# jibo27/3DGS_Hierarchical_Training

Measured on AMD Instinct MI355X. Metric: train-step images/sec + fwd+bwd ms @1M Gaussians, 980x545; 1/2/4/8 GPU, higher is better.
Workload: dtype f32

## Files before the change

### 3dgs_hierarchical_training_amd/csrc/gsr_kernels.hip

```cpp
#include <hip/hip_runtime.h>
#include <hip/hip_ext.h>
#include <type_traits>
#include <stdint.h>
#include <stdio.h>
#include <string.h>

#include <algorithm>
#include <atomic>
#include <chrono>
#include <cmath>
#include <map>
#include <mutex>
#include <tuple>
#include <vector>

#include "../../include/gsr.h"
#include "gsr_math.h"
#include "adam_math.h"
#include "radix_sort.h"
#include "blend_common.h"

#ifndef GSR_K9_UNROLL
#define GSR_K9_UNROLL 2
#endif
// ... 1073 lines not shown
#pragma unroll
        for (int g = 0; g < kDbMaxGroups; g++) v[g] = g < db.G ? db.GT[(size_t)g * db.Tp + t] : 0u;
#pragma unroll
        for (int g = 0; g < kDbMaxGroups; g++) {
            if (g < db.G) db.GT[(size_t)g * db.Tp + t] = tot;
            tot += v[g];
        }
    }
    if (t >= db.T) tot = 0u;
    const uint32_t inc = wave_inclusive_sum(tot);
    if (lane == 63) s_w[wave] = inc;
    __syncthreads();
    lo = s_lo[0] + s_lo[1] + s_lo[2] + s_lo[3];
    all = s_all[0] + s_all[1] + s_all[2] + s_all[3];
    uint32_t add = 0u;
#pragma unroll
    for (int w = 0; w < 4; w++) add += w < wave ? s_w[w] : 0u;
    const uint32_t base_t = (uint32_t)min(lo + add + inc - tot, 0xffffffffull);
    if (t < db.T) db.tbase[t] = base_t;
    if (cut.key) {
        if (t < db.T) {
            const uint32_t e = cut.cur[0] < (uint32_t)kVcEntries ? cut.cur[0] : 0u;
            const bool use = cut.enable && cut.cur[9] != 0u && cut.owner_n[e] == (uint32_t)db.N;
            uint32_t ck = (uint32_t)(db.NC - 1);
            const uint32_t k = use ? cut.key[(size_t)e * db.T + t] : kCutOpenKey;
            if (k != kCutOpenKey && k != 0u) {
                const float d = __uint_as_float(k);
                const uint32_t kc = __float_as_uint(fmaf(d, cut.margin, d));
                int a = 0, b = db.NC;
                while (a < b) { const int m = (a + b) >> 1; if (s_bkey[m] <= kc) a = m + 1; else b = m; }
                ck = (uint32_t)max(a - 1, 0);
            }
            cut.chunk[t] = (uint16_t)ck;
            cut.flag[t] = 0u;
            if (use) atomicAdd(&cut.hist[ck], 1u);
            if (t == 0) cut.ctl[3] = use ? 1u : 0u;
        }
    }
    if (slab == 0 && tid == 0) {
        db.tbase[db.T] = (uint32_t)min(all, 0xffffffffull);
        *total_out = all;
        if (host_out) {
            __atomic_store_n(host_out + 2, (unsigned long long)g_onesweep_giveups, __ATOMIC_RELAXED);
            __atomic_store_n(host_out + 3, (unsigned long long)(window_overflow ? *window_overflow : 0u), __ATOMIC_RELAXED);
            __atomic_store_n(host_out, all, __ATOMIC_RELAXED);
            __threadfence_system();
            __atomic_store_n(host_out + 1, host_seq, __ATOMIC_RELAXED);
            __threadfence_system();
        }
        if (late_out) scan_report_late(late_out, all, host_seq);
    }
}

constexpr int kDbPairs = 1024;
__device__ __forceinline__ void lds_order() { __builtin_amdgcn_fence(__ATOMIC_ACQ_REL, "wavefront"); __builtin_amdgcn_wave_barrier(); }

__device__ __forceinline__ uint32_t cut_frame(const ListCut& cut, const int NC, uint32_t& deep)
{
    const int lane = threadIdx.x & 63;
    deep = 0u;
    if (cut.ctl[3] == 0u) return (uint32_t)(NC - 1);
    constexpr int kR = 32;
    uint32_t v[kR];
#pragma unroll
    for (int q = 0; q < kR; q++) { const int c = NC - 1 - 64 * q - lane; v[q] = (64 * q < NC && c >= 0) ? cut.hist[c] : 0u; }
    uint32_t acc = 0u;
#pragma unroll
    for (int q = 0; q < kR; q++) {
        if (64 * q >= NC) break;
        const int c = NC - 1 - 64 * q - lane;
        const uint32_t inc = acc + wave_inclusive_sum(v[q]);
        const unsigned long long over = __ballot(c >= 0 && inc > (uint32_t)cut.dmax);
        if (over) {
            const int l = (int)__builtin_ctzll(over);
            deep = (uint32_t)__builtin_amdgcn_readlane((int)(inc - v[q]), l);
            return (uint32_t)(NC - 1 - 64 * q - l);
        }
        acc = (uint32_t)__builtin_amdgcn_readlane((int)inc, 63);
    }
    for (int top = NC - 1 - 64 * kR; top >= 0; top -= 64) {
        const int c = top - lane;
        const uint32_t w = c >= 0 ? cut.hist[c] : 0u;
        const uint32_t inc = acc + wave_inclusive_sum(w);
        const unsigned long long over = __ballot(c >= 0 && inc > (uint32_t)cut.dmax);
        if (over) {
            const int l = (int)__builtin_ctzll(over);
            deep = (uint32_t)__builtin_amdgcn_readlane((int)(inc - w), l);
            return (uint32_t)(top - l);
        }
        acc = (uint32_t)__builtin_amdgcn_readlane((int)inc, 63);
    }
    deep = acc;
    return 0u;
}

template <typename Want>
__device__ __forceinline__ void cut_chunk_tiles(const DirectBin& db, const int c, const int W, const int H, const int tiles_x, const int tiles_y,
                                                const uint32_t* __restrict__ sorted_gid, const TileRec* __restrict__ sorted_rec,
                                                const Splat* __restrict__ splat, uint32_t* __restrict__ list, const uint32_t cap,
                                                uint32_t* s_txy , uint32_t* s_pos , Want&& want)
{
    const int lane = threadIdx.x & 63;
    const unsigned long long lt = lanemask_lt();
    const int j0 = c * db.S, j1 = min(db.N, j0 + db.S);
    const uint32_t* gt = db.GT + (size_t)(c / db.Cg) * db.Tp;
    const uint16_t* mr = db.M + (size_t)c * db.Tp;
    auto load_rec = [&](int j) -> TileRec { TileRec r; r.mask = 0u; r.rect = 1u << 24; if (j < j1) r = sorted_rec[j]; return r; };
// ... 22 lines not shown
        }
        if (nt == 0) break;
        lds_order();
        TileRec rA = load_rec(j0 + lane), rB = load_rec(j0 + 64 + lane);
        uint32_t gA = load_gid(j0 + lane), gB = load_gid(j0 + 64 + lane);
        for (int j = j0; j < j1; j += 64) {
            const TileRec r = rA;
            const uint32_t g = gA;
            rA = rB; gA = gB;
            rB = load_rec(j + 128 + lane);
            gB = load_gid(j + 128 + lane);
            const bool big = (r.rect & kTileRecBig) != 0u && r.mask != 0u;
            const uint32_t ww = (r.rect >> 24) & 63u, rx0 = r.rect & 0xfffu, ry0 = (r.rect >> 12) & 0xfffu;
            TileTest tt = {};
            int bx0 = 0, by0 = 0, bx1 = 0, by1 = 0;
            if (big) {
                const Splat sp = splat[g];
                tile_rect_tight(sp.px, sp.py, sp.radius, sp.ca, sp.cb, sp.cc, sp.op, W, H, tiles_x, tiles_y, bx0, by0, bx1, by1);
                tt = make_tile_test(sp.px, sp.py, sp.ca, sp.cb, sp.cc, sp.op);
            }
            const bool any_big = __ballot(big) != 0ull;
            for (int k = 0; k < nt; k++) {
                const uint32_t txy = s_txy[k], tx = txy & 0xffffu, ty = txy >> 16;
                const uint32_t dx = tx - rx0, dy = ty - ry0, bit = dy * ww + dx;
                bool in = !big && dx < ww && bit < 32u && ((r.mask >> bit) & 1u) != 0u;
                if (any_big && big) in = (int)tx >= bx0 && (int)tx < bx1 && (int)ty >= by0 && (int)ty < by1 && tile_accept(tt, (int)tx, (int)ty, W, H);
                const unsigned long long b = __ballot(in);
                if (b == 0ull) continue;
                const uint32_t p0 = s_pos[k];
                if (in) { const uint32_t pos = p0 + (uint32_t)__popcll(b & lt); if (pos < cap) list[pos] = g; }
                lds_order();
                if (lane == 0) s_pos[k] = p0 + (uint32_t)__popcll(b);
                lds_order();
            }
        }
        lds_order();
    }
}

#ifdef GSR_DB_TIMING
__device__ unsigned long long g_db_dbg[16];
#define DB_T(k) do { const unsigned long long now_ = __builtin_readcyclecounter(); if (lane == 0) dbt[k] += now_ - dbt_last; dbt_last = now_; } while (0)
#else
#define DB_T(k) do { } while (0)
#endif
template <bool SLAB, bool PAIRS = false, int CUT = 0>
__global__ __launch_bounds__(64) void k_chunk_scatter(DirectBin db, int W, int H, int tiles_x, int tiles_y,
                                                      const uint32_t* __restrict__ sorted_gid, const TileRec* __restrict__ sorted_rec,
                                                      const Splat* __restrict__ splat, uint32_t* __restrict__ list, uint2* __restrict__ ranges,
                                                      uint32_t cap, const uint32_t* __restrict__ dkey = nullptr, uint2* __restrict__ pairs = nullptr,
                                                      ListCut cut = ListCut{})
{
    static_assert(!CUT || (!SLAB && !PAIRS), "the list cut serves the plain direct binning");
    extern __shared__ unsigned long long s_dyn[];
    const int LT = SLAB ? db.Tsp : db.Tp;
    unsigned long long* const s_mask = s_dyn;
    uint32_t* const s_cnt = reinterpret_cast<uint32_t*>(s_dyn + LT);
    uint32_t* const s_pair = s_cnt + LT;
    const int lane = threadIdx.x, b = (int)blockIdx.x;
    if (CUT == 2 && cut.ctl[2] == 0u) return;
    uint32_t cstar = 0u, ndeep = 0u;
    if (CUT == 1) cstar = cut_frame(cut, db.NC, ndeep);
    if (CUT == 2) cstar = cut.ctl[0];
    {
        const int t = b * 64 + lane;
        if (t < db.T) {
            uint32_t tend = db.tbase[t + 1];
            if (CUT == 1) {
                const uint32_t c1 = max((uint32_t)cut.chunk[t], cstar) + 1u;
                if (c1 < (uint32_t)db.NC) tend = db.tbase[t] + db.GT[(size_t)(c1 / (uint32_t)db.Cg) * db.Tp + t] + (uint32_t)db.M[(size_t)c1 * db.Tp + t];
                cut.tend[t] = tend;
            }
            const uint32_t lo = min(db.tbase[t], cap), hi = min(tend, cap);
            if (CUT != 2 || cut.flag[t]) ranges[t] = hi > lo ? make_uint2(lo, hi) : make_uint2(0u, 0u);
            if (CUT == 1) {
                const uint32_t e = cut.cur[0] < (uint32_t)kVcEntries ? cut.cur[0] : 0u;
                cut.key[(size_t)e * db.T + t] = 0u;
            }
        }
        if (CUT && b == 0 && lane == 0) {
            if (CUT == 1) {
                const uint32_t e = cut.cur[0] < (uint32_t)kVcEntries ? cut.cur[0] : 0u;
                cut.owner_n[e] = (uint32_t)db.N;
                cut.ctl[0] = cstar; cut.ctl[1] = ndeep;
                cut.stats[0] += 1u;
                cut.stats[3] += (uint32_t)(db.NC - 1) - min(cstar, (uint32_t)(db.NC - 1));
                cut.stats[4] += ndeep;
            } else { cut.stats[1] += 1u; cut.stats[2] += cut.ctl[2]; }
        }
    }
    const int per = (db.NC + 7) >> 3, kk = b >> 3, c = (b & 7) * per + (SLAB ? kk / db.NS : kk), slab = SLAB ? kk % db.NS : 0;
    if ((SLAB ? kk / db.NS : kk) >= per || c >= db.NC) return;
    if (CUT && (uint32_t)c > cstar) {
        if (CUT == 1 && ndeep == 0u) return;
        uint32_t* const s_tile = s_pair;
        uint32_t* const s_pos = s_pair + 64;
        if (CUT == 1) cut_chunk_tiles(db, c, W, H, tiles_x, tiles_y, sorted_gid, sorted_rec, splat, list, cap, s_tile, s_pos,
                                      [&](uint32_t t) { return (uint32_t)cut.chunk[t] >= (uint32_t)c; });
        else cut_chunk_tiles(db, c, W, H, tiles_x, tiles_y, sorted_gid, sorted_rec, splat, list, cap, s_tile, s_pos,
                             [&](uint32_t t) { return cut.flag[t] != 0u && (uint32_t)cut.chunk[t] < (uint32_t)c; });
        return;
    }
    if (CUT == 2) return;
    const uint32_t t0 = SLAB ? (uint32_t)(slab * db.Ts) : 0u;
    const uint32_t tn = SLAB ? (uint32_t)min(db.Ts, db.T - slab * db.Ts) : (uint32_t)db.T;
    const int srow0 = slab * db.slab_rows, srow1 = srow0 + db.slab_rows;
#ifdef GSR_DB_TIMING
    unsigned long long dbt[8] = {0, 0, 0, 0, 0, 0, 0, 0}, dbt_last = __builtin_readcyclecounter();
#endif
    {
        const uint32_t* gt = db.GT + (size_t)(c / db.Cg) * db.Tp;
        const uint16_t* mr = db.M + (size_t)c * db.Tp;
        constexpr int kRows = 36;
        for (int i0 = 0; i0 < LT; i0 += 64 * kRows) {
            uint32_t tb[kRows], gb[kRows], mc[kRows];
#pragma unroll
            for (int q = 0; q < kRows; q++) {
                const int i = i0 + 64 * q + lane;
                const bool v = i < LT && (uint32_t)i < tn + (SLAB ? 0u : (uint32_t)(db.Tp - db.T));
                const int g = (int)t0 + i;
                tb[q] = v && g < db.T ? db.tbase[g] : 0u;
                gb[q] = v ? gt[g] : 0u;
                mc[q] = v ? (uint32_t)mr[g] : 0u;
            }
#pragma unroll
            for (int q = 0; q < kRows; q++) {
                const int i = i0 + 64 * q + lane;
                if (i < LT) { s_cnt[i] = tb[q] + gb[q] + mc[q]; s_mask[i] = 0ull; }
            }
        }
    }
    lds_order();
    DB_T(0);
    const unsigned long long me = 1ull << lane, lt = lanemask_lt();
    const int j0 = c * db.S, j1 = min(db.N, j0 + db.S);
    auto load_gid = [&](int j) -> uint32_t { return j < j1 ? (PAIRS ? (uint32_t)j : sorted_gid[j]) : 0u; };
    auto load_rec = [&](int j) -> TileRec { TileRec r; r.mask = 0u; r.rect = 1u << 24; if (j < j1) r = sorted_rec[j]; return r; };
    auto load_key = [&](int j) -> uint32_t { return (PAIRS && j < j1) ? dkey[j] : 0u; };
    uint32_t gA = load_gid(j0 + lane), gB = load_gid(j0 + 64 + lane);
    TileRec rA = load_rec(j0 + lane), rB = load_rec(j0 + 64 + lane);
    uint32_t kA = load_key(j0 + lane), kB = load_key(j0 + 64 + lane);
    for (int j = j0 + lane; j - lane < j1; j += 64) {
        const uint32_t g = gA;
        TileRec r = rA;
        const uint32_t kd = kA;
        gA = gB; rA = rB; kA = kB;
        gB = load_gid(j + 128);
        rB = load_rec(j + 128);
        kB = load_key(j + 128);
        if (SLAB && !(r.rect & kTileRecBig)) {
            const int ww = (int)((r.rect >> 24) & 63u), ry0 = (int)((r.rect >> 12) & 0xfffu);
            const int lo = min(32, max(0, (srow0 - ry0) * ww)), hi = min(32, max(0, (srow1 - ry0) * ww));
            const uint32_t below_hi = hi >= 32 ? 0xffffffffu : ((1u << hi) - 1u), below_lo = lo >= 32 ? 0xffffffffu : ((1u << lo) - 1u);
            r.mask &= below_hi & ~below_lo;
        }
        const bool big = (r.rect & kTileRecBig) != 0u && r.mask != 0u, huge = big && (SLAB || r.mask > (uint32_t)kDbPairs);
        const unsigned long long bigs = __ballot(big && !huge), huges = __ballot(huge);
        const uint32_t cnt = huge ? 0u : tilerec_count(r);
        const uint32_t incl = wave_inclusive_sum(cnt);
        auto run_end = [&](int lo, uint32_t before) -> int {
            const unsigned long long over = __ballot(incl - before > (uint32_t)kDbPairs) & ~((1ull << lo) - 1ull);
            return over ? (int)__builtin_ctzll(over) : 64;
        };
        auto owners = [&](int lo, int hi, uint32_t before, bool with_or) {
            const bool mine = lane >= lo && lane < hi;
            if (!big && (with_or || mine)) {
                uint32_t* o = s_pair + (incl - cnt - before);
                small_rect_tiles(r, tiles_x, [&](uint32_t tg) {
                    const uint32_t t = tg - t0;
                    if (with_or) atomicOr(&s_mask[t], me);
                    if (mine) *o++ = (t << 6) | (uint32_t)lane;
                });
            }
            for (unsigned long long bm = bigs; bm != 0ull; bm &= bm - 1ull) {
                const int bl = (int)__builtin_ctzll(bm);
                const bool in_run = bl >= lo && bl < hi;
                if (!with_or && !in_run) continue;
                const uint32_t gg = (uint32_t)__builtin_amdgcn_readlane((int)g, bl), rect = (uint32_t)__builtin_amdgcn_readlane((int)r.rect, bl);
                uint32_t o = (uint32_t)__builtin_amdgcn_readlane((int)(incl - cnt), bl) - before;
                const Splat s = splat[gg];
                big_rect_tiles(s, rect, W, H, tiles_x, tiles_y, lane, [&](bool ok, uint32_t tg) {
                    const uint32_t t = tg - t0;
                    const unsigned long long acc = __ballot(ok);
                    if (ok) {
                        if (with_or) atomicOr(&s_mask[t], 1ull << bl);
                        if (in_run) s_pair[(o + (uint32_t)__popcll(acc & lt)) & (uint32_t)(kDbPairs - 1)] = (t << 6) | (uint32_t)bl;
                    }
                    o += (uint32_t)__popcll(acc);
                });
            }
        };
        int lo = 0, hi = run_end(0, 0u);
        uint32_t before = 0u;
        const bool one_run = hi == 64;
        DB_T(1);
        owners(0, hi, 0u, true);
        DB_T(2);
        for (unsigned long long bm = huges; bm != 0ull; bm &= bm - 1ull) {
            const int bl = (int)__builtin_ctzll(bm);
            const uint32_t gg = (uint32_t)__builtin_amdgcn_readlane((int)g, bl), rect = (uint32_t)__builtin_amdgcn_readlane((int)r.rect, bl);
            const Splat s = splat[gg];
            big_rect_tiles(s, rect, W, H, tiles_x, tiles_y, lane, [&](bool ok, uint32_t tg) { const uint32_t t = tg - t0; if (ok && t < tn) atomicOr(&s_mask[t], 1ull << bl); });
        }
        asm volatile("" : "+v"(gA), "+v"(rA.mask), "+v"(rA.rect));
        if (PAIRS) asm volatile("" : "+v"(kA));
        lds_order();
        DB_T(3);
        for (;;) {
            const uint32_t P = (uint32_t)__builtin_amdgcn_readlane((int)incl, hi - 1) - before;
            for (uint32_t p0 = 0u; p0 < P; p0 += 512u) {
                const uint32_t left = P - p0;
                auto batch = [&](auto rounds_tag) {
                    constexpr int RN = decltype(rounds_tag)::value;
                    uint32_t e[RN], go[RN], base[RN], ko[PAIRS ? RN : 1];
                    unsigned long long mk[RN];
#pragma unroll
                    for (int q = 0; q < RN; q++) e[q] = s_pair[(p0 + 64u * q + (uint32_t)lane) & (uint32_t)(kDbPairs - 1)];
#pragma unroll
                    for (int q = 0; q < RN; q++) {
                        const bool v = 64u * q + (uint32_t)lane < left;
                        e[q] = v ? e[q] : 0xffffffffu;
                        const uint32_t t = v ? e[q] >> 6 : 0u;
                        go[q] = (uint32_t)__builtin_amdgcn_ds_bpermute((int)((e[q] & 63u) << 2), (int)g);
                        if (PAIRS) ko[q] = (uint32_t)__builtin_amdgcn_ds_bpermute((int)((e[q] & 63u) << 2), (int)kd);
                        mk[q] = s_mask[t];
                        base[q] = s_cnt[t];
                    }
#pragma unroll
                    for (int q = 0; q < RN; q++)
                        if (e[q] != 0xffffffffu) {
                            const uint32_t pos = base[q] + (uint32_t)__popcll(mk[q] & ((1ull << (e[q] & 63u)) - 1ull));
                            if (pos < cap) {
                                if (PAIRS) pairs[pos] = make_uint2(ko[q], go[q]);
                                else list[pos] = go[q];
                            }
                        }
                };
                if (left <= 128u) batch(std::integral_constant<int, 2>{});
                else if (left <= 256u) batch(std::integral_constant<int, 4>{});
                else if (left <= 384u) batch(std::integral_constant<int, 6>{});
                else batch(std::integral_constant<int, 8>{});
            }
            if (hi == 64) break;
            lds_order();
            before += P;
            lo = hi;
            hi = run_end(lo, before);
            owners(lo, hi, before, false);
            lds_order();
        }
        for (unsigned long long bm = huges; bm != 0ull; bm &= bm - 1ull) {
            const int bl = (int)__builtin_ctzll(bm);
            const uint32_t gg = (uint32_t)__builtin_amdgcn_readlane((int)g, bl), rect = (uint32_t)__builtin_amdgcn_readlane((int)r.rect, bl);
            const Splat s = splat[gg];
            big_rect_tiles(s, rect, W, H, tiles_x, tiles_y, lane, [&](bool ok, uint32_t tg) {
                const uint32_t t = tg - t0;
                if (ok && t < tn) {
                    const uint32_t pos = s_cnt[t] + (uint32_t)__popcll(s_mask[t] & ((1ull << bl) - 1ull));
                    if (pos < cap) {
                        if (PAIRS) pairs[pos] = make_uint2((uint32_t)__builtin_amdgcn_readlane((int)kd, bl), gg);
                        else list[pos] = gg;
                    }
                }
            });
        }
        lds_order();
        DB_T(4);
        if (one_run) {
            const uint32_t P = (uint32_t)__builtin_amdgcn_readlane((int)incl, 63);
            for (uint32_t p0 = 0u; p0 < P; p0 += 512u) {
                const uint32_t left = P - p0;
                auto batch = [&](auto rounds_tag) {
                    constexpr int RN = decltype(rounds_tag)::value;
                    uint32_t e[RN];
#pragma unroll
                    for (int q = 0; q < RN; q++) e[q] = s_pair[(p0 + 64u * q + (uint32_t)lane) & (uint32_t)(kDbPairs - 1)];
#pragma unroll
                    for (int q = 0; q < RN; q++)
                        if (64u * q + (uint32_t)lane < left) { atomicAdd(&s_cnt[e[q] >> 6], 1u); s_mask[e[q] >> 6] = 0ull; }
                };
                if (left <= 128u) batch(std::integral_constant<int, 2>{});
                else if (left <= 256u) batch(std::integral_constant<int, 4>{});
                else if (left <= 384u) batch(std::integral_constant<int, 6>{});
                else batch(std::integral_constant<int, 8>{});
            }
        } else {
            if (!big) small_rect_tiles(r, tiles_x, [&](uint32_t tg) { const uint32_t t = tg - t0; atomicAdd(&s_cnt[t], 1u); s_mask[t] = 0ull; });
            for (unsigned long long bm = bigs; bm != 0ull; bm &= bm - 1ull) {
                const int bl = (int)__builtin_ctzll(bm);
                const uint32_t gg = (uint32_t)__builtin_amdgcn_readlane((int)g, bl), rect = (uint32_t)__builtin_amdgcn_readlane((int)r.rect, bl);
                const Splat s = splat[gg];
                big_rect_tiles(s, rect, W, H, tiles_x, tiles_y, lane, [&](bool ok, uint32_t tg) { const uint32_t t = tg - t0; if (ok && t < tn) { atomicAdd(&s_cnt[t], 1u); s_mask[t] = 0ull; } });
            }
        }
        for (unsigned long long bm = huges; bm != 0ull; bm &= bm - 1ull) {
            const int bl = (int)__builtin_ctzll(bm);
            const uint32_t gg = (uint32_t)__builtin_amdgcn_readlane((int)g, bl), rect = (uint32_t)__builtin_amdgcn_readlane((int)r.rect, bl);
            const Splat s = splat[gg];
            big_rect_tiles(s, rect, W, H, tiles_x, tiles_y, lane, [&](bool ok, uint32_t tg) { const uint32_t t = tg - t0; if (ok && t < tn) { atomicAdd(&s_cnt[t], 1u); s_mask[t] = 0ull; } });
        }
        lds_order();
        DB_T(5);
    }
#ifdef GSR_DB_TIMING
    if (lane == 0) {
        for (int k = 0; k < 6; k++) atomicAdd(&g_db_dbg[k], dbt[k]);
        atomicAdd(&g_db_dbg[6], 1ull);
        atomicAdd(&g_db_dbg[7], (unsigned long long)((j1 - j0 + 63) / 64));
    }
#endif
}

constexpr int kTsCap = 4096, kTsSmallMax = 1024;

template <int THREADS, int IPT, bool GATHER = false>
__device__ __forceinline__ void tile_sort_regs(const uint2* __restrict__ src, uint32_t* dst, uint32_t n, const uint32_t* __restrict__ dkey,
                                               unsigned long long (*s_mask)[256], uint32_t (*s_cnt)[256], uint32_t* s_keys, uint32_t* s_vals,
                                               uint32_t* s_start, uint32_t* s_wsum, uint32_t* s_bits)
{
    constexpr int WAVES = THREADS / 64;
    const int tid = threadIdx.x, wave = tid >> 6, lane = tid & 63;
    uint32_t key[IPT], val[IPT], dig[IPT], rnk[IPT];
    uint32_t k_or = 0u, k_and = 0xffffffffu;
#pragma unroll
    for (int r = 0; r < IPT; r++) {
        const uint32_t p = (uint32_t)(wave * (IPT * 64) + r * 64 + lane);
        if (GATHER) val[r] = p < n ? dst[p] : 0u;
        else if (p < n) { const uint2 e = src[p]; key[r] = e.x; val[r] = e.y; }
        if (!GATHER && p >= n) { key[r] = 0xffffffffu; val[r] = 0u; }
    }
    if (GATHER) {
#pragma unroll
        for (int r = 0; r < IPT; r++) {
            const uint32_t p = (uint32_t)(wave * (IPT * 64) + r * 64 + lane);
            key[r] = p < n ? dkey[val[r]] : 0xffffffffu;
        }
    }
#pragma unroll
    for (int r = 0; r < IPT; r++) {
        const uint32_t p = (uint32_t)(wave * (IPT * 64) + r * 64 + lane);
        if (p < n) { k_or |= key[r]; k_and &= key[r]; }
    }
#pragma unroll
    for (int off = 32; off > 0; off >>= 1) { k_or |= (uint32_t)__shfl_xor((int)k_or, off, 64); k_and &= (uint32_t)__shfl_xor((int)k_and, off, 64); }
    if (lane == 0) { s_bits[wave] = k_or; s_bits[WAVES + wave] = k_and; }
    __syncthreads();
    uint32_t differ = 0u;
    {
        uint32_t o = 0u, a = 0xffffffffu;
#pragma unroll
        for (int w = 0; w < WAVES; w++) { o |= s_bits[w]; a &= s_bits[WAVES + w]; }
        differ = o & ~a;
    }
#pragma unroll 1
// ... 2135 lines not shown
    if (!strcmp(name, "tile_sort")) { if (value < 0 || value > 2) return GSR_ERR_ARG; g_tile_sort = value; return GSR_OK; }
    if (!strcmp(name, "tile_sort_max_avg")) { if (value < 0) return GSR_ERR_ARG; g_tile_sort_max_avg = value; return GSR_OK; }
    if (!strcmp(name, "direct_slab_tiles")) { if (value < 0) return GSR_ERR_ARG; g_db_slab_tiles = value; return GSR_OK; }
    if (!strcmp(name, "view_pose_tol_e6")) { if (value < 0) return GSR_ERR_ARG; g_view_pose_tol_e6 = value; return GSR_OK; }
    if (!strcmp(name, "depth_sort9")) { g_depth_sort9 = value ? 1 : 0; return GSR_OK; }
    if (!strcmp(name, "direct_binning")) { g_direct_bin = value ? 1 : 0; return GSR_OK; }
    if (!strcmp(name, "speculative_binning")) { g_speculate = value ? 1 : 0; return GSR_OK; }
    if (!strcmp(name, "deterministic_backward")) { g_deterministic = value ? 1 : 0; return GSR_OK; }
    if (!strcmp(name, "binning_capacity_hint")) {
        std::lock_guard<std::mutex> lk(g_state_mutex);
        g_hint_override = value > 0 ? value : -1;
        return GSR_OK;
    }
    if (!strcmp(name, "reset_speculation")) {
        std::lock_guard<std::mutex> lk(g_state_mutex);
        g_hints.clear(); g_hint_override = -1;
        g_spec_overflows = 0; g_spec_forwards = 0; g_exact_forwards = 0; g_depth_window_resorts = 0;
        g_full_depth_sort.clear();
        return GSR_OK;
    }
    if (!strcmp(name, "profile")) { g_profile = (value == 2 || value == 3) ? value : (value ? 1 : 0); g_profile_tick = 0; return GSR_OK; }
    if (!strcmp(name, "prep_hist_max_n")) { g_prep_hist_max_n = value; return GSR_OK; }
    if (!strcmp(name, "small_sort9")) { if (value < 0) return GSR_ERR_ARG; g_small_sort9 = value; return GSR_OK; }
    if (!strcmp(name, "poll_iters")) { g_poll_iters = value < 0 ? 0 : value; return GSR_OK; }
    if (!strcmp(name, "emit_hist")) { g_emit_hist = value ? 1 : 0; return GSR_OK; }
    if (!strcmp(name, "sort_algo")) { if (value < 0 || value > 2) return GSR_ERR_ARG; g_sort_algo = value; return GSR_OK; }
    if (!strcmp(name, "blend_bwd_ppt")) {
        if (value < 0 || value > 2) return GSR_ERR_ARG;
        g_bwd_ppt = value; return GSR_OK;
    }
    return GSR_ERR_ARG;
}

struct DirectBinScratch { size_t M, GT, tbase, bsum, cut_chunk, cut_tend, cut_flag, cut_ctl, cut_bkey, cut_hist, bytes; };
static bool direct_bin_geometry(int N, int T, DirectBin& db, DirectBinScratch& ds, int tiles_x = 0, int tile_rows = 0)
{
    if (N < 1 || T < 1) return false;
    db.NS = 1; db.Ts = 0; db.Tsp = 0; db.slab_rows = 0;
    static const bool force_slabs = getenv("GSR_DB_FORCE_SLABS") != nullptr;
    if (T > kDbMaxTiles || (force_slabs && g_db_slab_tiles > 0 && tiles_x > 0 && tile_rows > 0 && tiles_x * tile_rows == T)) {
        if (g_db_slab_tiles <= 0 || tiles_x <= 0 || tile_rows <= 0 || tiles_x * tile_rows != T || tiles_x > kDbMaxTiles || T > 32768) return false;
        const int rows = std::max(1, std::min(g_db_slab_tiles, kDbMaxTiles) / tiles_x);
        db.slab_rows = rows; db.Ts = rows * tiles_x; db.Tsp = (db.Ts + 63) & ~63; db.NS = (tile_rows + rows - 1) / rows;
        if (db.NS > 16) return false;
    }
    static std::atomic<int> cus_cached{0};
    int cus = cus_cached.load(std::memory_order_relaxed);
    if (!cus) {
        int dev = 0, n = 0;
        cus = (hipGetDevice(&dev) == hipSuccess && hipDeviceGetAttribute(&n, hipDeviceAttributeMultiprocessorCount, dev) == hipSuccess && n > 0) ? n : 256;
        cus_cached.store(cus, std::memory_order_relaxed);
    }
    db.N = N; db.T = T; db.Tp = (T + 63) & ~63;
    const int lds = 12 * (db.NS > 1 ? db.Tsp : db.Tp) + 4 * kDbPairs;
    const char* env = getenv("GSR_DB_WAVES_PER_CU");
    int per_cu = std::min(16, (160 * 1024) / lds);
    if (env && atoi(env) > 0) per_cu = atoi(env);
    const long long resident = std::max<long long>(1, (long long)cus * per_cu / db.NS);
    const char* env_s = getenv("GSR_DB_MIN_CHUNK");
    const int min_s = env_s && atoi(env_s) > 0 ? atoi(env_s) : 128;
    long long S = ((long long)N + resident - 1) / resident;
    S = std::max<long long>(min_s, (S + 63) & ~63ll);
    if (S > 65472) return false;
    db.S = (int)S;
    db.NC = (int)(((long long)N + S - 1) / S);
    int G = 1;
    while (G * G < db.NC) G++;
    db.Cg = std::max(1, std::min((db.NC + G - 1) / G, 65535 / db.S));
    db.G = (db.NC + db.Cg - 1) / db.Cg;
    if (db.G > kDbMaxGroups) return false;
    size_t o = 0;
    ds.M = o; o += align256((size_t)db.NC * db.Tp * sizeof(uint16_t));
    ds.GT = o; o += align256((size_t)db.G * db.Tp * sizeof(uint32_t));
    ds.tbase = o; o += align256((size_t)(db.Tp + 1) * sizeof(uint32_t));
    ds.bsum = o; o += align256((size_t)db.G * ((db.Tp + 255) / 256) * sizeof(uint32_t));
    ds.cut_chunk = o; o += align256((size_t)db.Tp * sizeof(uint16_t));
    ds.cut_tend = o; o += align256((size_t)db.Tp * sizeof(uint32_t));
    ds.cut_flag = o; o += align256((size_t)db.Tp * sizeof(uint32_t));
    ds.cut_ctl = o; o += 256;
    ds.cut_bkey = o; o += align256((size_t)db.NC * sizeof(uint32_t));
    ds.cut_hist = o; o += align256((size_t)db.NC * sizeof(uint32_t));
    ds.bytes = o;
    return true;
}

int gsr_forward(const GsrForwardArgs* a, GsrForwardOut* out, void* stream_)
{
    CallTimer call_timer(g_fwd_calls, g_fwd_ns);
    hipStream_t st = (hipStream_t)stream_;
    if (!a || !out) return fail(GSR_ERR_ARG, "null args%s");
    int rc = check_common(a->N, a->M, a->D, a->W, a->H);
    if (rc) return rc;
    if (!a->out_color || !a->out_depth || !a->out_alpha || !a->image || !a->bg || !a->alloc)
        return fail(GSR_ERR_ARG, "missing output / workspace pointer%s");
    const int N = a->N, W = a->W, H = a->H;
    BatchDev bt;
    rc = batch_dev(a->batch, N, H, bt);
    if (rc) return rc;
    const int NB = bt.B;
    const int opt_ppt = g_blend_ppt ? g_blend_ppt : 7, opt_map = g_tile_map, opt_ckpt = g_ckpt_first;
    const int tiles_x = (W + kTile - 1) / kTile, tiles_y = (H + kTile - 1) / kTile, T = tiles_x * tiles_y * NB;
    if (NB > 1 && opt_ppt < 6) return fail(GSR_ERR_ARG, "batch: served by the default forward blend kernel only%s");
    if (a->out_color_clamped && opt_ppt < 6) return fail(GSR_ERR_ARG, "out_color_clamped: served by the default forward blend kernel only%s");
    out->num_rendered = 0; out->binning = nullptr; out->binning_bytes = 0; out->binning_capacity = 0;
    out->forward_flags = pack_fwd_flags(opt_ppt, opt_map, opt_ckpt);
    uint64_t R = 0;
    BlendBalance bb = {};
// ... 46 lines not shown
    auto launch_binning_t = [&](auto key_tag, uint64_t capacity, const unsigned long long* n_dev, bool prezeroed) -> int {
        using KeyT = decltype(key_tag);
        if (!prezeroed) GSR_HIP(hipMemsetAsync(ranges, 0, (size_t)T * sizeof(uint2), st));
        if (capacity == 0) return GSR_OK;
        KeyT* tkey = reinterpret_cast<KeyT*>(bs + S.tile);
        KeyT* tkey_alt = reinterpret_cast<KeyT*>(bs + S.tile_alt);
        uint32_t* gid_alt2 = reinterpret_cast<uint32_t*>(bs + S.gid_alt);
        uint32_t* block_sums = reinterpret_cast<uint32_t*>(fs + L.block_sums);
        uint32_t* v0 = (tile_passes & 1) ? gid_alt2 : list;
        uint32_t* v1 = (tile_passes & 1) ? list : gid_alt2;
        const bool emit_hist = g_sort_algo == 2 && prezeroed && g_emit_hist;
        EmitHist eh = {};
        if (emit_hist) {
            eh.ghist = reinterpret_cast<uint32_t*>(bs + S.sort);
            eh.status = onesweep_status(bs + S.sort);
            eh.status_words = onesweep_status_words<KeyT>((uint32_t)capacity, bits);
            eh.bits = bits;
            eh.n_dev = n_dev;
        }
        {
            ProfScope ps(P_EMIT, st);
            hipLaunchKernelGGL(k_emit<KeyT>, dim3(nb), dim3(kEmitThreads), 0, st, N, W, H, tiles_x, tiles_y, sorted_gid, splat,
                               tsort ? ts_rec : reinterpret_cast<const TileRec*>(fs + L.srec), block_sums, tkey, v0,
                               (uint32_t)capacity, eh);
        }
        int in_alt = 0;
        {
            ProfScope ps(P_SORT_TILE, st);
            GSR_HIP(g_sort_algo == 2 ? onesweep_sort_pairs<KeyT>(tkey, v0, tkey_alt, v1, (uint32_t)capacity, 0, bits, bs + S.sort,
                                                                 &in_alt, st, n_dev, prezeroed, emit_hist)
                                     : radix_sort_pairs<KeyT>(tkey, v0, tkey_alt, v1, (uint32_t)capacity, 0, tile_passes * 8, bs + S.sort,
                                                              &in_alt, st));
        }
        const KeyT* skey = in_alt ? tkey_alt : tkey;
        {
            ProfScope ps(P_RANGES, st);
            constexpr uint32_t kpb = 256u * (16u / (uint32_t)sizeof(KeyT));
            hipLaunchKernelGGL(k_tile_ranges<KeyT>, dim3(((uint32_t)capacity + kpb - 1) / kpb), dim3(256), 0, st, (uint32_t)capacity, skey, ranges, n_dev);
        }
        if (tsort) {
            ProfScope ps(P_SORT_DEPTH, st);
            hipLaunchKernelGGL(k_tile_sort_wave<true>, dim3(T), dim3(64), 0, st, ranges, pairs, list, T, ts_dkey);
            hipLaunchKernelGGL((k_tile_sort<1024, true>), dim3(std::min(T, 512)), dim3(1024), 0, st, ranges, pairs, pairs_alt, list, T, ts_dkey);
        }
        return GSR_OK;
    };
    auto launch_binning = [&](uint64_t capacity, const unsigned long long* n_dev, bool prezeroed) -> int {
        if (direct) {
            if (capacity == 0) { GSR_HIP(hipMemsetAsync(ranges, 0, (size_t)T * sizeof(uint2), st)); return GSR_OK; }
            const int per = (db.NC + 7) / 8, grid = std::max(8 * per * db.NS, (T + 63) / 64);
            if (tsort) {
                {
                    ProfScope ps(P_EMIT, st);
                    hipLaunchKernelGGL((k_chunk_scatter<false, true>), dim3(grid), dim3(64), (size_t)12 * db.Tp + 4 * kDbPairs, st, db, W, H, tiles_x, tiles_y,
                                       (const uint32_t*)nullptr, ts_rec, splat, list, ranges, (uint32_t)std::min<uint64_t>(capacity, 0xffffffffull), ts_dkey, pairs);
                }
                ProfScope ps2(P_SORT_TILE, st);
                hipLaunchKernelGGL(k_tile_sort_wave<false>, dim3(T), dim3(64), 0, st, ranges, pairs, list, T, (const uint32_t*)nullptr);
                hipLaunchKernelGGL(k_tile_sort<1024>, dim3(std::min(T, 512)), dim3(1024), 0, st, ranges, pairs, pairs_alt, list, T);
                return GSR_OK;
            }
            ProfScope ps(P_EMIT, st);
            if (db.NS > 1)
                hipLaunchKernelGGL(k_chunk_scatter<true>, dim3(grid), dim3(64), (size_t)12 * db.Tsp + 4 * kDbPairs, st, db, W, H, tiles_x, tiles_y, sorted_gid,
                                   reinterpret_cast<const TileRec*>(fs + L.srec), splat, list, ranges, (uint32_t)std::min<uint64_t>(capacity, 0xffffffffull));
            else if (lc.key) {
                lc_capacity = capacity;
                hipLaunchKernelGGL((k_chunk_scatter<false, false, 1>), dim3(grid), dim3(64), (size_t)12 * db.Tp + 4 * kDbPairs, st, db, W, H,
                                   tiles_x, tiles_y, sorted_gid, reinterpret_cast<const TileRec*>(fs + L.srec), splat, list, ranges,
                                   (uint32_t)std::min<uint64_t>(capacity, 0xffffffffull), (const uint32_t*)nullptr, (uint2*)nullptr, lc);
            } else
                hipLaunchKernelGGL(k_chunk_scatter<false>, dim3(grid), dim3(64), (size_t)12 * db.Tp + 4 * kDbPairs, st, db, W, H, tiles_x, tiles_y, sorted_gid,
                                   reinterpret_cast<const TileRec*>(fs + L.srec), splat, list, ranges, (uint32_t)std::min<uint64_t>(capacity, 0xffffffffull));
            return GSR_OK;
        }
        return wide_keys ? launch_binning_t(uint32_t{}, capacity, n_dev, prezeroed) : launch_binning_t(uint16_t{}, capacity, n_dev, prezeroed);
    };
    auto launch_blend = [&](bool prezeroed) -> int {
        const int ppt = opt_ppt;
        if (!prezeroed) GSR_HIP(hipMemsetAsync(staged, 0, (size_t)T * 16, st));
        float* ckpt = reinterpret_cast<float*>(bin + B.ckpt);
        if (ppt == 7 && g_profile && (g_profile != 3 || g_profile_tick.fetch_add(1u) % 3u == 0u)) {
            hipEvent_t ea = nullptr, eb = nullptr;
            if (hipEventCreate(&ea) != hipSuccess || hipEventCreate(&eb) != hipSuccess) return fail(GSR_ERR_HIP, "hipEventCreate failed%s");
            hipExtLaunchKernelGGL(k_blend_fwd_w6<true>, dim3(8 * 4 * slots_per_xcd(opt_map, T, tiles_x)), dim3(64), 0, st, ea, eb, 0, W, H, tiles_x, T, ranges, list,
                                  splat, a->bg, a->out_color, a->out_depth, a->out_alpha, img, staged, opt_map, ckpt, opt_ckpt, tiles_y, bb, a->out_color_clamped,
                                  lc, lc.key ? 1 : 0);
            std::lock_guard<std::mutex> lk(g_prof_mutex);
            g_prof_events[P_BLEND_FWD].push_back({ea, eb});
        } else {
            ProfScope ps(ppt == 7 && g_profile == 3 ? P_COUNT : P_BLEND_FWD, st);
            if (ppt == 7)
                hipLaunchKernelGGL(k_blend_fwd_w6<true>, dim3(8 * 4 * slots_per_xcd(opt_map, T, tiles_x)), dim3(64), 0, st, W, H, tiles_x, T, ranges, list, splat, a->bg,
                                   a->out_color, a->out_depth, a->out_alpha, img, staged, opt_map, ckpt, opt_ckpt, tiles_y, bb, a->out_color_clamped,
                                   lc, lc.key ? 1 : 0);
            else if (ppt == 6)
                hipLaunchKernelGGL(k_blend_fwd_w6<false>, dim3(8 * 4 * slots_per_xcd(opt_map, T, tiles_x)), dim3(64), 0, st, W, H, tiles_x, T, ranges, list, splat, a->bg,
                                   a->out_color, a->out_depth, a->out_alpha, img, staged, opt_map, ckpt, opt_ckpt, tiles_y, BlendBalance{}, a->out_color_clamped);
            else return fail(GSR_ERR_ARG, "unknown forward blend variant%s");
        }
        if (ppt == 7 && lc.key && lc_capacity > 0) {
            ProfScope ps(P_CUT_REPAIR, st);
            const int per = (db.NC + 7) / 8, grid = std::max(8 * per * db.NS, (T + 63) / 64);
            hipLaunchKernelGGL((k_chunk_scatter<false, false, 2>), dim3(grid), dim3(64), (size_t)12 * db.Tp + 4 * kDbPairs, st, db, W, H,
                               tiles_x, tiles_y, sorted_gid, reinterpret_cast<const TileRec*>(fs + L.srec), splat, list, ranges,
                               (uint32_t)std::min<uint64_t>(lc_capacity, 0xffffffffull), (const uint32_t*)nullptr, (uint2*)nullptr, lc);
            hipLaunchKernelGGL(k_blend_fwd_w6<true>, dim3(8 * 4 * slots_per_xcd(opt_map, T, tiles_x)), dim3(64), 0, st, W, H, tiles_x, T, ranges, list, splat, a->bg,
                               a->out_color, a->out_depth, a->out_alpha, img, staged, opt_map, ckpt, opt_ckpt, tiles_y, bb, a->out_color_clamped, lc, 2);
        }
        GSR_HIP(hipGetLastError());
        return GSR_OK;
    };

    if (N == 0) {
        rc = alloc_binning(0);
        if (rc) return rc;
        rc = launch_binning(0, nullptr, false);
        if (rc) return rc;
        rc = launch_blend(false);
        if (rc) return rc;
        out->binning = bin;
        out->binning_bytes = B.bytes;
        return GSR_OK;
    }

    if (!a->means3D || !a->opacities || !a->geom || !a->radii || !a->viewmatrix || !a->projmatrix)
        return fail(GSR_ERR_ARG, "missing input pointer%s");
    if ((a->shs == nullptr) == (a->colors_precomp == nullptr)) return fail(GSR_ERR_ARG, "provide exactly one of shs / colors_precomp%s");
    if ((a->cov3D_precomp == nullptr) == (a->scales == nullptr || a->rotations == nullptr))
        return fail(GSR_ERR_ARG, "provide exactly one of (scales, rotations) / cov3D_precomp%s");
    if (a->shs && (!a->campos || a->M < (a->D + 1) * (a->D + 1))) return fail(GSR_ERR_ARG, "shs needs campos and M >= (D+1)^2%s");

    int dev_id = 0;
    GSR_HIP(hipGetDevice(&dev_id));
    const auto hint_key = std::make_tuple(dev_id, W, H * NB, n_bucket(N));
    uint64_t hint = 0;
    {
        std::lock_guard<std::mutex> lk(g_state_mutex);
        if (g_hint_override > 0) { hint = (uint64_t)g_hint_override; g_hint_override = -1; }
        else { auto it = g_hints.find(hint_key); if (it != g_hints.end()) hint = it->second; }
    }
    const bool speculative = g_speculate && g_sort_algo == 2 && hint > 0;
    const uint64_t cap = speculative ? hint : 0;
    {
        const int ts_mode = g_tile_sort;
        const uint64_t avg = (hint > 0 ? hint : (uint64_t)N * 4u) / (uint64_t)T;
        const bool auto_ok = ts_mode == 1 && avg <= (uint64_t)g_tile_sort_max_avg && (direct || N / std::max(1, NB) <= g_tile_sort_emit_max_n);
        tsort = (ts_mode == 2 || auto_ok) && g_sort_algo == 2 && (direct ? (NB == 1 && db.NS == 1) : true);
    }

    fs = static_cast<uint8_t*>(a->alloc(align256(L.bytes) + (direct ? dbs.bytes : 0), GSR_ALLOC_SCRATCH, a->alloc_user));
    if (!fs) return fail(GSR_ERR_ALLOC, "scratch allocation failed%s");
    if (speculative) {
        rc = alloc_binning(cap);
        if (rc) return rc;
    }
    uint32_t* dkey = reinterpret_cast<uint32_t*>(fs + L.dkey);
// ... 644 lines not shown
```

Before: 1206.

## Use 32-bit per-tile lane masks and per-run half-wave placement in chunk scatter

The direct-binning scatter kernel replaces its 64-bit per-tile lane mask with a 32-bit mask and processes each run of pairs in two half-wave passes. The OR-mask is now built inside each run rather than once for the whole wave. The pair buffer shrinks from 1024 to 512 entries, and the per-workgroup LDS footprint drops from 12*LT+4K to 8*LT+2K bytes. The intent is higher occupancy (more waves per CU) and cheaper 32-bit LDS atomics, at the cost of extra barriers and a repeated huge-splat tile walk per half.

```diff
diff --git a/3dgs_hierarchical_training_amd/csrc/gsr_kernels.hip b/3dgs_hierarchical_training_amd/csrc/gsr_kernels.hip
--- a/3dgs_hierarchical_training_amd/csrc/gsr_kernels.hip
+++ b/3dgs_hierarchical_training_amd/csrc/gsr_kernels.hip
@@ -1149,7 +1149,8 @@
     }
 }
 
-constexpr int kDbPairs = 1024;
+constexpr int kDbPairs = 512;
+__host__ __device__ constexpr size_t db_scatter_lds(int LT) { return (size_t)8 * LT + 4 * kDbPairs; }
 __device__ __forceinline__ void lds_order() { __builtin_amdgcn_fence(__ATOMIC_ACQ_REL, "wavefront"); __builtin_amdgcn_wave_barrier(); }
 
 __device__ __forceinline__ uint32_t cut_frame(const ListCut& cut, const int NC, uint32_t& deep)
@@ -1278,10 +1279,10 @@
                                                       ListCut cut = ListCut{})
 {
     static_assert(!CUT || (!SLAB && !PAIRS), "the list cut serves the plain direct binning");
-    extern __shared__ unsigned long long s_dyn[];
+    extern __shared__ uint32_t s_dyn[];
     const int LT = SLAB ? db.Tsp : db.Tp;
-    unsigned long long* const s_mask = s_dyn;
-    uint32_t* const s_cnt = reinterpret_cast<uint32_t*>(s_dyn + LT);
+    uint32_t* const s_mask = s_dyn;
+    uint32_t* const s_cnt = s_dyn + LT;
     uint32_t* const s_pair = s_cnt + LT;
     const int lane = threadIdx.x, b = (int)blockIdx.x;
     if (CUT == 2 && cut.ctl[2] == 0u) return;
@@ -1352,13 +1353,13 @@
 #pragma unroll
             for (int q = 0; q < kRows; q++) {
                 const int i = i0 + 64 * q + lane;
-                if (i < LT) { s_cnt[i] = tb[q] + gb[q] + mc[q]; s_mask[i] = 0ull; }
+                if (i < LT) { s_cnt[i] = tb[q] + gb[q] + mc[q]; s_mask[i] = 0u; }
             }
         }
     }
     lds_order();
     DB_T(0);
-    const unsigned long long me = 1ull << lane, lt = lanemask_lt();
+    const unsigned long long lt = lanemask_lt();
     const int j0 = c * db.S, j1 = min(db.N, j0 + db.S);
     auto load_gid = [&](int j) -> uint32_t { return j < j1 ? (PAIRS ? (uint32_t)j : sorted_gid[j]) : 0u; };
     auto load_rec = [&](int j) -> TileRec { TileRec r; r.mask = 0u; r.rect = 1u << 24; if (j < j1) r = sorted_rec[j]; return r; };
@@ -1384,148 +1385,123 @@
         const unsigned long long bigs = __ballot(big && !huge), huges = __ballot(huge);
         const uint32_t cnt = huge ? 0u : tilerec_count(r);
         const uint32_t incl = wave_inclusive_sum(cnt);
+        auto lanes = [](int lo, int hi) -> unsigned long long { return (hi >= 64 ? ~0ull : ((1ull << hi) - 1ull)) & ~((1ull << lo) - 1ull); };
         auto run_end = [&](int lo, uint32_t before) -> int {
             const unsigned long long over = __ballot(incl - before > (uint32_t)kDbPairs) & ~((1ull << lo) - 1ull);
             return over ? (int)__builtin_ctzll(over) : 64;
         };
-        auto owners = [&](int lo, int hi, uint32_t before, bool with_or) {
-            const bool mine = lane >= lo && lane < hi;
-            if (!big && (with_or || mine)) {
+        auto owners = [&](int lo, int hi, uint32_t before) {
+            if (!big && lane >= lo && lane < hi) {
                 uint32_t* o = s_pair + (incl - cnt - before);
-                small_rect_tiles(r, tiles_x, [&](uint32_t tg) {
-                    const uint32_t t = tg - t0;
-                    if (with_or) atomicOr(&s_mask[t], me);
-                    if (mine) *o++ = (t << 6) | (uint32_t)lane;
-                });
-            }
-            for (unsigned long long bm = bigs; bm != 0ull; bm &= bm - 1ull) {
+                small_rect_tiles(r, tiles_x, [&](uint32_t tg) { *o++ = ((tg - t0) << 6) | (uint32_t)lane; });
+            }
+            for (unsigned long long bm = bigs & lanes(lo, hi); bm != 0ull; bm &= bm - 1ull) {
                 const int bl = (int)__builtin_ctzll(bm);
-                const bool in_run = bl >= lo && bl < hi;
-                if (!with_or && !in_run) continue;
                 const uint32_t gg = (uint32_t)__builtin_amdgcn_readlane((int)g, bl), rect = (uint32_t)__builtin_amdgcn_readlane((int)r.rect, bl);
                 uint32_t o = (uint32_t)__builtin_amdgcn_readlane((int)(incl - cnt), bl) - before;
                 const Splat s = splat[gg];
                 big_rect_tiles(s, rect, W, H, tiles_x, tiles_y, lane, [&](bool ok, uint32_t tg) {
                     const uint32_t t = tg - t0;
                     const unsigned long long acc = __ballot(ok);
-                    if (ok) {
-                        if (with_or) atomicOr(&s_mask[t], 1ull << bl);
-                        if (in_run) s_pair[(o + (uint32_t)__popcll(acc & lt)) & (uint32_t)(kDbPairs - 1)] = (t << 6) | (uint32_t)bl;
-                    }
+                    if (ok) s_pair[(o + (uint32_t)__popcll(acc & lt)) & (uint32_t)(kDbPairs - 1)] = (t << 6) | (uint32_t)bl;
                     o += (uint32_t)__popcll(acc);
                 });
             }
         };
-        int lo = 0, hi = run_end(0, 0u);
-        uint32_t before = 0u;
-        const bool one_run = hi == 64;
-        DB_T(1);
-        owners(0, hi, 0u, true);
-        DB_T(2);
-        for (unsigned long long bm = huges; bm != 0ull; bm &= bm - 1ull) {
-            const int bl = (int)__builtin_ctzll(bm);
-            const uint32_t gg = (uint32_t)__builtin_amdgcn_readlane((int)g, bl), rect = (uint32_t)__builtin_amdgcn_readlane((int)r.rect, bl);
-            const Splat s = splat[gg];
-            big_rect_tiles(s, rect, W, H, tiles_x, tiles_y, lane, [&](bool ok, uint32_t tg) { const uint32_t t = tg - t0; if (ok && t < tn) atomicOr(&s_mask[t], 1ull << bl); });
-        }
-        asm volatile("" : "+v"(gA), "+v"(rA.mask), "+v"(rA.rect));
-        if (PAIRS) asm volatile("" : "+v"(kA));
-        lds_order();
-        DB_T(3);
-        for (;;) {
+        auto huge_walk = [&](unsigned long long hm, auto&& f) {
+            for (; hm != 0ull; hm &= hm - 1ull) {
+                const int bl = (int)__builtin_ctzll(hm);
+                const uint32_t gg = (uint32_t)__builtin_amdgcn_readlane((int)g, bl), rect = (uint32_t)__builtin_amdgcn_readlane((int)r.rect, bl);
+                const Splat s = splat[gg];
+                big_rect_tiles(s, rect, W, H, tiles_x, tiles_y, lane, [&](bool ok, uint32_t tg) { const uint32_t t = tg - t0; if (ok && t < tn) f(t, bl, gg); });
+            }
+        };
+        auto place_run = [&](int lo, int hi, uint32_t before) {
             const uint32_t P = (uint32_t)__builtin_amdgcn_readlane((int)incl, hi - 1) - before;
-            for (uint32_t p0 = 0u; p0 < P; p0 += 512u) {
-                const uint32_t left = P - p0;
-                auto batch = [&](auto rounds_tag) {
-                    constexpr int RN = decltype(rounds_tag)::value;
-                    uint32_t e[RN], go[RN], base[RN], ko[PAIRS ? RN : 1];
-                    unsigned long long mk[RN];
-#pragma unroll
-                    for (int q = 0; q < RN; q++) e[q] = s_pair[(p0 + 64u * q + (uint32_t)lane) & (uint32_t)(kDbPairs - 1)];
+            const unsigned long long run = lanes(lo, hi);
+            auto batch = [&](auto rounds_tag) {
+                constexpr int RN = decltype(rounds_tag)::value;
+                uint32_t e[RN], go[RN], ko[PAIRS ? RN : 1];
+#pragma unroll
+                for (int q = 0; q < RN; q++) e[q] = s_pair[(64u * q + (uint32_t)lane) & (uint32_t)(kDbPairs - 1)];
+#pragma unroll
+                for (int q = 0; q < RN; q++) {
+                    e[q] = 64u * q + (uint32_t)lane < P ? e[q] : 0xffffffffu;
+                    go[q] = (uint32_t)__builtin_amdgcn_ds_bpermute((int)((e[q] & 63u) << 2), (int)g);
+                    if (PAIRS) ko[q] = (uint32_t)__builtin_amdgcn_ds_bpermute((int)((e[q] & 63u) << 2), (int)kd);
+                }
+#pragma unroll
+                for (int h = 0; h < 2; h++) {
+                    const unsigned long long half = h ? 0xffffffff00000000ull : 0x00000000ffffffffull;
+                    if ((run & half) == 0ull) continue;
+                    const unsigned long long hm = huges & run & half;
+                    bool act[RN];
+                    uint32_t t[RN], mk[RN], base[RN];
 #pragma unroll
                     for (int q = 0; q < RN; q++) {
-                        const bool v = 64u * q + (uint32_t)lane < left;
-                        e[q] = v ? e[q] : 0xffffffffu;
-                        const uint32_t t = v ? e[q] >> 6 : 0u;
-                        go[q] = (uint32_t)__builtin_amdgcn_ds_bpermute((int)((e[q] & 63u) << 2), (int)g);
-                        if (PAIRS) ko[q] = (uint32_t)__builtin_amdgcn_ds_bpermute((int)((e[q] & 63u) << 2), (int)kd);
-                        mk[q] = s_mask[t];
-                        base[q] = s_cnt[t];
+                        act[q] = e[q] != 0xffffffffu && ((e[q] >> 5) & 1u) == (uint32_t)h;
+                        t[q] = act[q] ? e[q] >> 6 : 0u;
+                        if (act[q]) atomicOr(&s_mask[t[q]], 1u << (e[q] & 31u));
                     }
+                    if (hm) huge_walk(hm, [&](uint32_t tt, int bl, uint32_t) { atomicOr(&s_mask[tt], 1u << (bl & 31)); });
+                    lds_order();
+#pragma unroll
+                    for (int q = 0; q < RN; q++) { mk[q] = s_mask[t[q]]; base[q] = s_cnt[t[q]]; }
 #pragma unroll
                     for (int q = 0; q < RN; q++)
-                        if (e[q] != 0xffffffffu) {
-                            const uint32_t pos = base[q] + (uint32_t)__popcll(mk[q] & ((1ull << (e[q] & 63u)) - 1ull));
+                        if (act[q]) {
+                            const uint32_t pos = base[q] + (uint32_t)__popc(mk[q] & ((1u << (e[q] & 31u)) - 1u));
                             if (pos < cap) {
                                 if (PAIRS) pairs[pos] = make_uint2(ko[q], go[q]);
                                 else list[pos] = go[q];
                             }
                         }
-                };
-                if (left <= 128u) batch(std::integral_constant<int, 2>{});
-                else if (left <= 256u) batch(std::integral_constant<int, 4>{});
-                else if (left <= 384u) batch(std::integral_constant<int, 6>{});
-                else batch(std::integral_constant<int, 8>{});
-            }
-            if (hi == 64) break;
+                    if (hm) {
+                        huge_walk(hm, [&](uint32_t tt, int bl, uint32_t gg) {
+                            const uint32_t pos = s_cnt[tt] + (uint32_t)__popc(s_mask[tt] & ((1u << (bl & 31)) - 1u));
+                            if (pos < cap) {
+                                if (PAIRS) pairs[pos] = make_uint2((uint32_t)__builtin_amdgcn_readlane((int)kd, bl), gg);
+                                else list[pos] = gg;
+                            }
+                        });
+                        lds_order();
+#pragma unroll
+                        for (int q = 0; q < RN; q++)
+                            if (act[q]) { atomicAdd(&s_cnt[t[q]], 1u); s_mask[t[q]] = 0u; }
+                        huge_walk(hm, [&](uint32_t tt, int, uint32_t) { atomicAdd(&s_cnt[tt], 1u); s_mask[tt] = 0u; });
+                    } else {
+                        lds_order();
+#pragma unroll
+                        for (int q = 0; q < RN; q++)
+                            if (act[q] && (mk[q] >> (e[q] & 31u)) == 1u) { s_cnt[t[q]] = base[q] + (uint32_t)__popc(mk[q]); s_mask[t[q]] = 0u; }
+                    }
+                    lds_order();
+                }
+            };
+            static_assert(kDbPairs == 512, "one batch of at most 8 rounds holds the whole buffer");
+            if (P <= 128u) batch(std::integral_constant<int, 2>{});
+            else if (P <= 256u) batch(std::integral_constant<int, 4>{});
+            else if (P <= 384u) batch(std::integral_constant<int, 6>{});
+            else batch(std::integral_constant<int, 8>{});
+        };
+        int hi = run_end(0, 0u);
+        DB_T(1);
+        owners(0, hi, 0u);
+        DB_T(2);
+        asm volatile("" : "+v"(gA), "+v"(rA.mask), "+v"(rA.rect));
+        if (PAIRS) asm volatile("" : "+v"(kA));
+        lds_order();
+        DB_T(3);
+        place_run(0, hi, 0u);
+        DB_T(4);
+        while (hi < 64) {
+            const uint32_t before = (uint32_t)__builtin_amdgcn_readlane((int)incl, hi - 1);
+            const int lo = hi;
+            hi = run_end(lo, before);
+            owners(lo, hi, before);
             lds_order();
-            before += P;
-            lo = hi;
-            hi = run_end(lo, before);
-            owners(lo, hi, before, false);
-            lds_order();
-        }
-        for (unsigned long long bm = huges; bm != 0ull; bm &= bm - 1ull) {
-            const int bl = (int)__builtin_ctzll(bm);
-            const uint32_t gg = (uint32_t)__builtin_amdgcn_readlane((int)g, bl), rect = (uint32_t)__builtin_amdgcn_readlane((int)r.rect, bl);
-            const Splat s = splat[gg];
-            big_rect_tiles(s, rect, W, H, tiles_x, tiles_y, lane, [&](bool ok, uint32_t tg) {
-                const uint32_t t = tg - t0;
-                if (ok && t < tn) {
-                    const uint32_t pos = s_cnt[t] + (uint32_t)__popcll(s_mask[t] & ((1ull << bl) - 1ull));
-                    if (pos < cap) {
-                        if (PAIRS) pairs[pos] = make_uint2((uint32_t)__builtin_amdgcn_readlane((int)kd, bl), gg);
-                        else list[pos] = gg;
-                    }
-                }
-            });
-        }
-        lds_order();
-        DB_T(4);
-        if (one_run) {
-            const uint32_t P = (uint32_t)__builtin_amdgcn_readlane((int)incl, 63);
-            for (uint32_t p0 = 0u; p0 < P; p0 += 512u) {
-                const uint32_t left = P - p0;
-                auto batch = [&](auto rounds_tag) {
-                    constexpr int RN = decltype(rounds_tag)::value;
-                    uint32_t e[RN];
-#pragma unroll
-                    for (int q = 0; q < RN; q++) e[q] = s_pair[(p0 + 64u * q + (uint32_t)lane) & (uint32_t)(kDbPairs - 1)];
-#pragma unroll
-                    for (int q = 0; q < RN; q++)
-                        if (64u * q + (uint32_t)lane < left) { atomicAdd(&s_cnt[e[q] >> 6], 1u); s_mask[e[q] >> 6] = 0ull; }
-                };
-                if (left <= 128u) batch(std::integral_constant<int, 2>{});
-                else if (left <= 256u) batch(std::integral_constant<int, 4>{});
-                else if (left <= 384u) batch(std::integral_constant<int, 6>{});
-                else batch(std::integral_constant<int, 8>{});
-            }
-        } else {
-            if (!big) small_rect_tiles(r, tiles_x, [&](uint32_t tg) { const uint32_t t = tg - t0; atomicAdd(&s_cnt[t], 1u); s_mask[t] = 0ull; });
-            for (unsigned long long bm = bigs; bm != 0ull; bm &= bm - 1ull) {
-                const int bl = (int)__builtin_ctzll(bm);
-                const uint32_t gg = (uint32_t)__builtin_amdgcn_readlane((int)g, bl), rect = (uint32_t)__builtin_amdgcn_readlane((int)r.rect, bl);
-                const Splat s = splat[gg];
-                big_rect_tiles(s, rect, W, H, tiles_x, tiles_y, lane, [&](bool ok, uint32_t tg) { const uint32_t t = tg - t0; if (ok && t < tn) { atomicAdd(&s_cnt[t], 1u); s_mask[t] = 0ull; } });
-            }
-        }
-        for (unsigned long long bm = huges; bm != 0ull; bm &= bm - 1ull) {
-            const int bl = (int)__builtin_ctzll(bm);
-            const uint32_t gg = (uint32_t)__builtin_amdgcn_readlane((int)g, bl), rect = (uint32_t)__builtin_amdgcn_readlane((int)r.rect, bl);
-            const Splat s = splat[gg];
-            big_rect_tiles(s, rect, W, H, tiles_x, tiles_y, lane, [&](bool ok, uint32_t tg) { const uint32_t t = tg - t0; if (ok && t < tn) { atomicAdd(&s_cnt[t], 1u); s_mask[t] = 0ull; } });
-        }
-        lds_order();
+            place_run(lo, hi, before);
+        }
         DB_T(5);
     }
 #ifdef GSR_DB_TIMING
@@ -3767,7 +3743,7 @@
         cus_cached.store(cus, std::memory_order_relaxed);
     }
     db.N = N; db.T = T; db.Tp = (T + 63) & ~63;
-    const int lds = 12 * (db.NS > 1 ? db.Tsp : db.Tp) + 4 * kDbPairs;
+    const int lds = (int)db_scatter_lds(db.NS > 1 ? db.Tsp : db.Tp);
     const char* env = getenv("GSR_DB_WAVES_PER_CU");
     int per_cu = std::min(16, (160 * 1024) / lds);
     if (env && atoi(env) > 0) per_cu = atoi(env);
@@ -3920,7 +3896,7 @@
             if (tsort) {
                 {
                     ProfScope ps(P_EMIT, st);
-                    hipLaunchKernelGGL((k_chunk_scatter<false, true>), dim3(grid), dim3(64), (size_t)12 * db.Tp + 4 * kDbPairs, st, db, W, H, tiles_x, tiles_y,
+                    hipLaunchKernelGGL((k_chunk_scatter<false, true>), dim3(grid), dim3(64), db_scatter_lds(db.Tp), st, db, W, H, tiles_x, tiles_y,
                                        (const uint32_t*)nullptr, ts_rec, splat, list, ranges, (uint32_t)std::min<uint64_t>(capacity, 0xffffffffull), ts_dkey, pairs);
                 }
                 ProfScope ps2(P_SORT_TILE, st);
@@ -3930,15 +3906,15 @@
             }
             ProfScope ps(P_EMIT, st);
             if (db.NS > 1)
-                hipLaunchKernelGGL(k_chunk_scatter<true>, dim3(grid), dim3(64), (size_t)12 * db.Tsp + 4 * kDbPairs, st, db, W, H, tiles_x, tiles_y, sorted_gid,
+                hipLaunchKernelGGL(k_chunk_scatter<true>, dim3(grid), dim3(64), db_scatter_lds(db.Tsp), st, db, W, H, tiles_x, tiles_y, sorted_gid,
                                    reinterpret_cast<const TileRec*>(fs + L.srec), splat, list, ranges, (uint32_t)std::min<uint64_t>(capacity, 0xffffffffull));
             else if (lc.key) {
                 lc_capacity = capacity;
-                hipLaunchKernelGGL((k_chunk_scatter<false, false, 1>), dim3(grid), dim3(64), (size_t)12 * db.Tp + 4 * kDbPairs, st, db, W, H,
+                hipLaunchKernelGGL((k_chunk_scatter<false, false, 1>), dim3(grid), dim3(64), db_scatter_lds(db.Tp), st, db, W, H,
                                    tiles_x, tiles_y, sorted_gid, reinterpret_cast<const TileRec*>(fs + L.srec), splat, list, ranges,
                                    (uint32_t)std::min<uint64_t>(capacity, 0xffffffffull), (const uint32_t*)nullptr, (uint2*)nullptr, lc);
             } else
-                hipLaunchKernelGGL(k_chunk_scatter<false>, dim3(grid), dim3(64), (size_t)12 * db.Tp + 4 * kDbPairs, st, db, W, H, tiles_x, tiles_y, sorted_gid,
+                hipLaunchKernelGGL(k_chunk_scatter<false>, dim3(grid), dim3(64), db_scatter_lds(db.Tp), st, db, W, H, tiles_x, tiles_y, sorted_gid,
                                    reinterpret_cast<const TileRec*>(fs + L.srec), splat, list, ranges, (uint32_t)std::min<uint64_t>(capacity, 0xffffffffull));
             return GSR_OK;
         }
@@ -3970,7 +3946,7 @@
         if (ppt == 7 && lc.key && lc_capacity > 0) {
             ProfScope ps(P_CUT_REPAIR, st);
             const int per = (db.NC + 7) / 8, grid = std::max(8 * per * db.NS, (T + 63) / 64);
-            hipLaunchKernelGGL((k_chunk_scatter<false, false, 2>), dim3(grid), dim3(64), (size_t)12 * db.Tp + 4 * kDbPairs, st, db, W, H,
+            hipLaunchKernelGGL((k_chunk_scatter<false, false, 2>), dim3(grid), dim3(64), db_scatter_lds(db.Tp), st, db, W, H,
                                tiles_x, tiles_y, sorted_gid, reinterpret_cast<const TileRec*>(fs + L.srec), splat, list, ranges,
                                (uint32_t)std::min<uint64_t>(lc_capacity, 0xffffffffull), (const uint32_t*)nullptr, (uint2*)nullptr, lc);
             hipLaunchKernelGGL(k_blend_fwd_w6<true>, dim3(8 * 4 * slots_per_xcd(opt_map, T, tiles_x)), dim3(64), 0, st, W, H, tiles_x, T, ranges, list, splat, a->bg,
```

Result: no change. 1216, median of 6 (+0.8%).
